# luxfi/tfhe

Measured on AMD Instinct MI355X. Metric: PBS/sec at TFHE 128-bit default (N=1024), batch=4096; 1/2/4/8 MI355X, higher is better.
Workload: dtype f64

## Files before the change

tfhe_amd/csrc/api.cpp:

```cpp
#include <dlfcn.h>
#include <hip/hip_runtime_api.h>
#include <rccl/rccl.h>
#include <stdarg.h>
#include <stdio.h>
#include <stdlib.h>
#include <string.h>

#include <algorithm>
#include <memory>
#include <mutex>
#include <string>
#include <thread>
#include <vector>

#include "../../include/tfhe_hip.h"
#include "client.h"
#include "gl64.h"
#include "pbs_kernels.h"

using tfhe::u32;
using tfhe::u64;

namespace {

// ... 54 lines not shown
}

struct Rccl {
  bool tried = false, ok = false;
  std::string why;
  ncclResult_t (*comm_init_all)(ncclComm_t*, int, const int*) = nullptr;
  ncclResult_t (*bcast)(const void*, void*, size_t, ncclDataType_t, int, ncclComm_t, hipStream_t) = nullptr;
  ncclResult_t (*group_start)() = nullptr;
  ncclResult_t (*group_end)() = nullptr;
  ncclResult_t (*comm_destroy)(ncclComm_t) = nullptr;
  const char* (*err)(ncclResult_t) = nullptr;
};

Rccl& rccl() {
  static Rccl r;
  static std::mutex m;
  std::lock_guard<std::mutex> lk(m);
  if (r.tried) return r;
  r.tried = true;
  void* h = dlopen("librccl.so.1", RTLD_NOW | RTLD_NOLOAD);
  if (!h) h = dlopen("librccl.so.1", RTLD_NOW | RTLD_LOCAL);
  if (!h) h = dlopen("/opt/rocm/lib/librccl.so.1", RTLD_NOW | RTLD_LOCAL);
  if (!h) {
    r.why = std::string("dlopen librccl.so.1: ") + dlerror();
    return r;
  }
  r.comm_init_all = (decltype(r.comm_init_all))dlsym(h, "ncclCommInitAll");
  r.bcast = (decltype(r.bcast))dlsym(h, "ncclBroadcast");
  r.group_start = (decltype(r.group_start))dlsym(h, "ncclGroupStart");
  r.group_end = (decltype(r.group_end))dlsym(h, "ncclGroupEnd");
  r.comm_destroy = (decltype(r.comm_destroy))dlsym(h, "ncclCommDestroy");
  r.err = (decltype(r.err))dlsym(h, "ncclGetErrorString");
  r.ok = r.comm_init_all && r.bcast && r.group_start && r.group_end && r.comm_destroy && r.err;
  if (!r.ok) r.why = "librccl.so.1 lacks ncclCommInitAll / ncclBroadcast / ncclGroupStart / ncclGroupEnd";
  return r;
}

struct DeviceGuard {
  int prev = -1;
  explicit DeviceGuard(int dev) {
    if (hipGetDevice(&prev) != hipSuccess) prev = -1;
    if (prev != dev) (void)hipSetDevice(dev);
  }
  ~DeviceGuard() {
    int cur = -1;
    if (prev >= 0 && hipGetDevice(&cur) == hipSuccess && cur != prev) (void)hipSetDevice(prev);
  }
};

}

struct tfhe_shard {
  int device = 0;
  hipStream_t stream = nullptr;
  u64* d_bsk = nullptr;
  u64* d_ksk = nullptr;
  void* d_ks_planes = nullptr;
  u64* d_tw = nullptr;
  u64* d_ms_zeros = nullptr;
  u64* d_big = nullptr;
  size_t big_cap = 0;
  void* d_stage = nullptr;
  size_t stage_cap = 0;
  void* d_ks_dig = nullptr;
  size_t ks_dig_cap = 0;
  hipEvent_t ws_free = nullptr;
  hipStream_t ws_last = nullptr;
  bool ws_used = false;
  std::vector<hipEvent_t> ev[3];
  std::vector<hipEvent_t> ev_pool;
};

struct tfhe_ctx {
  tfhe_params p{};
  std::vector<tfhe_shard> sh;
  bool keys = false;
  bool ks_valu = false;
  size_t lat_max = 1024;
  u64 ninv = 0;
  uint32_t ms_count = 0;
  double ms_bound = 0, ms_r_sigma = 0, ms_var128 = 0;
  int bcast_mode = 0;
  std::vector<ncclComm_t> comms;
  std::mutex mu;
  bool timing = false;
};

namespace {

using shard = tfhe_shard;

int grow(shard& s, void** ptr, size_t* cap, size_t bytes) {
  if (*cap >= bytes) return 0;
  if (s.ws_used) HIP_TRY(hipEventSynchronize(s.ws_free));
  if (*ptr) (void)hipFree(*ptr);
  *ptr = nullptr;
  *cap = 0;
  HIP_TRY(hipMalloc(ptr, bytes));
  *cap = bytes;
  return 0;
}

int ws_begin(shard& s, hipStream_t st) {
  if (s.ws_used && s.ws_last != st) HIP_TRY(hipStreamWaitEvent(st, s.ws_free, 0));
  return 0;
}
int ws_end(shard& s, hipStream_t st) {
  HIP_TRY(hipEventRecord(s.ws_free, st));
  s.ws_last = st;
  s.ws_used = true;
  return 0;
}

hipEvent_t take_event(shard& s) {
  if (!s.ev_pool.empty()) {
    hipEvent_t e = s.ev_pool.back();
    s.ev_pool.pop_back();
    return e;
  }
  hipEvent_t e = nullptr;
  if (hipEventCreate(&e) != hipSuccess) return nullptr;
  return e;
}

void timed_begin(tfhe_ctx* c, shard& s, int which, hipStream_t st) {
  if (!c->timing) return;
  hipEvent_t e = take_event(s);
  if (e) {
    (void)hipEventRecord(e, st);
    s.ev[which].push_back(e);
  }
}
void timed_end(tfhe_ctx* c, shard& s, int which, hipStream_t st) {
  if (!c->timing) return;
  if (s.ev[which].size() % 2 == 0) return;
  hipEvent_t e = take_event(s);
  if (e) {
    (void)hipEventRecord(e, st);
    s.ev[which].push_back(e);
  } else {
    s.ev_pool.push_back(s.ev[which].back());
    s.ev[which].pop_back();
  }
}

uint32_t io_dim(const tfhe_params& p) { return p.order == 0 ? p.n : p.k * p.N; }

hipError_t launch_br(tfhe_ctx* c, shard& s, const u64* in, size_t B, const u64* luts, const u32* idx, size_t n_lut,
                     u64* out_big, u64* out_acc, hipStream_t st) {
  if (is_fft(c->p) && c->p.N == 2048)
    return tfhe::launch_blind_rotate_fft2k(in, B, (int)c->p.n, luts, idx, (int)n_lut, (const double*)s.d_bsk,
                                           (const double*)s.d_tw, out_big, out_acc, st, c->lat_max);
  if (is_fft(c->p))
    return tfhe::launch_blind_rotate_fft(in, B, (int)c->p.n, luts, idx, (int)n_lut, (const double*)s.d_bsk,
                                         (const double*)s.d_tw, out_big, out_acc, st, c->lat_max);
  if (c->p.N == 2048)
    return tfhe::launch_blind_rotate_2048(in, B, (int)c->p.n, luts, idx, (int)n_lut, s.d_bsk, s.d_tw, out_big, out_acc,
                                          st, c->lat_max);
  return tfhe::launch_blind_rotate(in, B, (int)c->p.n, luts, idx, (int)n_lut, s.d_bsk, s.d_tw, out_big, out_acc, st,
                                   c->lat_max);
}

uint32_t log2u(uint32_t x) {
  uint32_t l = 0;
  while ((1u << l) < x) l++;
  return l;
}

hipError_t launch_ms(tfhe_ctx* c, shard& s, u64* small, size_t B, int* picks, hipStream_t st) {
  return tfhe::launch_ms_reduce(small, B, (int)c->p.n, s.d_ms_zeros, (int)c->ms_count, (int)log2u(2 * c->p.N),
                                c->ms_bound, c->ms_r_sigma, c->ms_var128, picks, st);
}

int launch_ks(tfhe_ctx* c, shard& s, const u64* in_big, size_t B, u64* out, hipStream_t st) {
  const int big_dim = (int)(c->p.k * c->p.N);
  if (c->ks_valu || !s.d_ks_planes) {
    HIP_TRY(tfhe::launch_keyswitch(in_big, B, big_dim, s.d_ksk, (int)c->p.n, (int)c->p.ks_base_log,
                                   (int)c->p.ks_level, out, st));
    return 0;
  }
  RC_TRY(grow(s, &s.d_ks_dig, &s.ks_dig_cap, tfhe::ks_digits_bytes(B, big_dim, (int)c->p.ks_level)));
  HIP_TRY(tfhe::launch_keyswitch_mfma(in_big, B, big_dim, s.d_ks_planes, (int)c->p.n, (int)c->p.ks_base_log,
                                      (int)c->p.ks_level, s.d_ks_dig, out, st));
  return 0;
}

int pbs_device(tfhe_ctx* c, shard& s, const u64* d_in, size_t B, const u64* d_luts, size_t n_lut, const u32* d_idx,
               u64* d_out, hipStream_t st) {
  const size_t big = (size_t)c->p.k * c->p.N + 1, small = (size_t)c->p.n + 1;
  RC_TRY(grow(s, (void**)&s.d_big, &s.big_cap, B * (c->p.order == 0 ? big : small) * sizeof(u64)));
  if (c->p.order == 0) {
    timed_begin(c, s, 0, st);
    HIP_TRY(launch_br(c, s, d_in, B, d_luts, d_idx, n_lut, s.d_big, nullptr, st));
    timed_end(c, s, 0, st);
    timed_begin(c, s, 1, st);
    RC_TRY(launch_ks(c, s, s.d_big, B, d_out, st));
    timed_end(c, s, 1, st);
  } else {
    timed_begin(c, s, 1, st);
    RC_TRY(launch_ks(c, s, d_in, B, s.d_big, st));
    timed_end(c, s, 1, st);
    if (c->ms_count) {
      timed_begin(c, s, 2, st);
      HIP_TRY(launch_ms(c, s, s.d_big, B, nullptr, st));
      timed_end(c, s, 2, st);
    }
    timed_begin(c, s, 0, st);
    HIP_TRY(launch_br(c, s, s.d_big, B, d_luts, d_idx, n_lut, d_out, nullptr, st));
// ... 128 lines not shown
      DeviceGuard g(c->sh[i].device);
      r = R->bcast(i == 0 ? (const void*)src : (const void*)dst[i], i == 0 ? (void*)src : (void*)dst[i], count,
                   ncclUint64, 0, c->comms[i], c->sh[i].stream);
    }
    const ncclResult_t r2 = R->group_end();
    if (r != ncclSuccess || r2 != ncclSuccess)
      return fail(TFHE_HIP_EDEVICE, "ncclBroadcast: %s", R->err(r != ncclSuccess ? r : r2));
    for (int i = 0; i < nd; i++) {
      DeviceGuard g(c->sh[i].device);
      HIP_TRY(hipStreamSynchronize(c->sh[i].stream));
    }
    c->bcast_mode = 2;
    return 0;
  }
  if (mode == 0) return 0;
  for (int k = 0; k < ncalls; k++) {
    shard& s = c->sh[calls[k]];
    DeviceGuard g(s.device);
    if (s.device == c->sh[0].device)
      HIP_TRY(hipMemcpyAsync(dst[calls[k]], src, count * 8, hipMemcpyDeviceToDevice, s.stream));
    else
      HIP_TRY(hipMemcpyPeerAsync(dst[calls[k]], s.device, src, c->sh[0].device, count * 8, s.stream));
    HIP_TRY(hipStreamSynchronize(s.stream));
  }
  c->bcast_mode = 1;
  return 0;
}

int convert_keys(tfhe_ctx* c, shard& s, const u64* std_bsk, size_t bsk_len) {
  const size_t polys = bsk_len / c->p.N;
  DeviceGuard g(s.device);
  if (!c->ks_valu) {
    const int big_dim = (int)(c->p.k * c->p.N);
    if (!s.d_ks_planes)
      HIP_TRY(hipMalloc(&s.d_ks_planes, tfhe::ks_planes_bytes(big_dim, (int)c->p.ks_level, (int)c->p.n)));
    HIP_TRY(tfhe::launch_ksk_planes(s.d_ksk, big_dim, (int)c->p.ks_level, (int)c->p.n, s.d_ks_planes, s.stream));
  }
  if (is_fft(c->p) && c->p.N == 2048)
    HIP_TRY(tfhe::launch_bsk_to_fourier2k(std_bsk, (double*)s.d_bsk, polys, (const double*)s.d_tw, s.stream));
  else if (is_fft(c->p))
    HIP_TRY(tfhe::launch_bsk_to_fourier(std_bsk, (double*)s.d_bsk, polys, (const double*)s.d_tw, s.stream));
  else if (c->p.N == 2048)
    HIP_TRY(tfhe::launch_bsk_to_ntt_2048(std_bsk, s.d_bsk, polys, s.d_tw, c->ninv, s.stream));
  else
    HIP_TRY(tfhe::launch_bsk_to_ntt(std_bsk, s.d_bsk, (int)(polys / 12), s.d_tw, c->ninv, s.stream));
  HIP_TRY(hipStreamSynchronize(s.stream));
  return 0;
}

int shard_init(tfhe_ctx* c, shard& s) {
  DeviceGuard g(s.device);
  HIP_TRY(hipStreamCreateWithFlags(&s.stream, hipStreamNonBlocking));
  HIP_TRY(hipEventCreateWithFlags(&s.ws_free, hipEventDisableTiming));
  const tfhe_params& p = c->p;
  using namespace tfhe;
  if (is_fft(p)) {
    std::vector<double> tw(p.N == 2048 ? fft2k_tables_len() : fft_tables_len());
    if (p.N == 2048) make_fft2k_tables(tw.data());
    else make_fft_tables(tw.data());
    if (!fft_slot_constants_ok() || !fft2k_slot_constants_ok())
      return fail(TFHE_HIP_EUNSUPPORTED, "FFT64: compile-time twist constants differ from the host tables");
    HIP_TRY(hipMalloc(&s.d_tw, tw.size() * 8));
    HIP_TRY(hipMemcpy(s.d_tw, tw.data(), tw.size() * 8, hipMemcpyHostToDevice));
    return 0;
  }
  std::vector<u64> tw(p.N == 2048 ? ntt2048_tables_len() : 4 * p.N);
  if (p.N == 2048) make_ntt2048_tables(canonical_psi(p.N), tw.data());
  else make_ntt_tables(canonical_psi(p.N), tw.data());
  HIP_TRY(hipMalloc(&s.d_tw, tw.size() * 8));
  HIP_TRY(hipMemcpy(s.d_tw, tw.data(), tw.size() * 8, hipMemcpyHostToDevice));
  return 0;
}

void shard_free(shard& s) {
  DeviceGuard g(s.device);
  if (s.stream) (void)hipStreamSynchronize(s.stream);
  for (int w = 0; w < 3; w++)
    for (auto e : s.ev[w]) (void)hipEventDestroy(e);
  for (auto e : s.ev_pool) (void)hipEventDestroy(e);
  (void)hipFree(s.d_bsk);
  (void)hipFree(s.d_ksk);
  (void)hipFree(s.d_ks_planes);
  (void)hipFree(s.d_ks_dig);
  (void)hipFree(s.d_tw);
  (void)hipFree(s.d_ms_zeros);
  (void)hipFree(s.d_big);
  (void)hipFree(s.d_stage);
  if (s.ws_free) (void)hipEventDestroy(s.ws_free);
  if (s.stream) (void)hipStreamDestroy(s.stream);
}

template <class F>
int for_each_slice(tfhe_ctx* c, size_t B, F&& fn) {
  const size_t nd = c->sh.size();
  std::vector<int> rc(nd, 0);
  std::vector<std::string> msg(nd);
  auto run = [&](size_t i) {
    const size_t lo = B * i / nd, hi = B * (i + 1) / nd;
    if (lo == hi) return;
    DeviceGuard g(c->sh[i].device);
    rc[i] = fn(i, lo, hi);
    if (rc[i]) msg[i] = g_err;
  };
  if (nd == 1) {
    run(0);
    return rc[0];
// ... 635 lines not shown
```

tfhe_amd/csrc/fft512.h:

```cpp
#pragma once
#pragma clang fp contract(off)
#include <hip/hip_runtime.h>

#include "gl64.h"
#include "ntt1024.h"

namespace tfhe {
namespace fftk {

constexpr int M = 512;
constexpr int S1 = 72, S2 = 65;
constexpr int T_C64 = 576;
constexpr int TW_TWIST = 0, TW_A = 512, TW_B = 1024, TW_I = 1536, TW_C64 = 2048;
constexpr double SQRT1_2 = 0.70710678118654752440;

#ifndef FFT_LDS_WAIT
#define FFT_LDS_WAIT 1
#endif
__device__ __forceinline__ void lds_order() {
#if FFT_LDS_WAIT
  wave_lds_sync();
#else
  __builtin_amdgcn_fence(__ATOMIC_ACQ_REL, "wavefront");
#endif
// ... 309 lines not shown
  for (int e = 0; e < 8; e++) {
    const double2 v = T[tb.b1 + 8 * e];
    xr[e] = v.x;
    xi[e] = v.y;
  }
  lds_order();
  dft8<false>(xr, xi);
#pragma unroll
  for (int e = 1; e < 8; e++) cmul<false>(xr[e], xi[e], wb[e]);
#pragma unroll
  for (int e = 0; e < 8; e++) T[lane + S2 * e] = make_double2(xr[e], xi[e]);
  lds_order();
#pragma unroll
  for (int e = 0; e < 8; e++) {
    const double2 v = T[tb.b2 + e];
    xr[e] = v.x;
    xi[e] = v.y;
  }
  lds_order();
  dft8<false>(xr, xi);
}

__device__ __forceinline__ void dft512_inv_rb(double (&xr)[8], double (&xi)[8], double2* T, int lane, TBase tb,
                                              const double2 (&wb)[8], const double2* twI) {
  dft8<true>(xr, xi);
#pragma unroll
  for (int e = 1; e < 8; e++) cmul<true>(xr[e], xi[e], wb[e]);
#pragma unroll
  for (int e = 0; e < 8; e++) T[tb.b2 + e] = make_double2(xr[e], xi[e]);
  lds_order();
#pragma unroll
  for (int e = 0; e < 8; e++) {
    const double2 v = T[lane + S2 * e];
    xr[e] = v.x;
    xi[e] = v.y;
  }
  lds_order();
  dft8<true>(xr, xi);
#pragma unroll
  for (int e = 0; e < 8; e++) cmul<true>(xr[e], xi[e], twI[64 * e + lane]);
#pragma unroll
  for (int e = 0; e < 8; e++) T[tb.b1 + 8 * e] = make_double2(xr[e], xi[e]);
  lds_order();
#pragma unroll
  for (int e = 0; e < 8; e++) {
    const double2 v = T[lane + S1 * e];
    xr[e] = v.x;
    xi[e] = v.y;
  }
  lds_order();
  dft8<true>(xr, xi);
}

template <bool TWIN = false, int BSTR = 8>
__device__ __forceinline__ void dft512_fwd_c(double (&xr)[8], double (&xi)[8], double2* T, int lane, TBase tb,
                                             const double2* twAl, const double2* twBc) {
  if constexpr (TWIN) twist_dft8_fwd(xr, xi);
  else dft8<false>(xr, xi);
#pragma unroll
  for (int e = 0; e < 8; e++) cmul<false>(xr[e], xi[e], twAl[64 * e]);
#pragma unroll
  for (int e = 0; e < 8; e++) T[lane + S1 * e] = make_double2(xr[e], xi[e]);
  lds_order();
#pragma unroll
  for (int e = 0; e < 8; e++) {
    const double2 v = T[tb.b1 + 8 * e];
    xr[e] = v.x;
    xi[e] = v.y;
  }
  lds_order();
  dft8<false>(xr, xi);
#pragma unroll
  for (int e = 1; e < 8; e++) cmul<false>(xr[e], xi[e], twBc[BSTR * e]);
#pragma unroll
  for (int e = 0; e < 8; e++) T[lane + S2 * e] = make_double2(xr[e], xi[e]);
  lds_order();
#pragma unroll
  for (int e = 0; e < 8; e++) {
    const double2 v = T[tb.b2 + e];
    xr[e] = v.x;
    xi[e] = v.y;
  }
  lds_order();
  dft8<false>(xr, xi);
}

template <int BSTR = 8>
__device__ __forceinline__ void dft512_inv_c(double (&xr)[8], double (&xi)[8], double2* T, int lane, TBase tb,
                                             const double2* twBc, const double2* twIl) {
  dft8<true>(xr, xi);
#pragma unroll
  for (int e = 1; e < 8; e++) cmul<true>(xr[e], xi[e], twBc[BSTR * e]);
#pragma unroll
  for (int e = 0; e < 8; e++) T[tb.b2 + e] = make_double2(xr[e], xi[e]);
  lds_order();
#pragma unroll
  for (int e = 0; e < 8; e++) {
    const double2 v = T[lane + S2 * e];
    xr[e] = v.x;
    xi[e] = v.y;
  }
  lds_order();
  dft8<true>(xr, xi);
#pragma unroll
  for (int e = 0; e < 8; e++) cmul<true>(xr[e], xi[e], twIl[64 * e]);
#pragma unroll
// ... 223 lines not shown
```

tfhe_amd/csrc/pbs_fft.hip:

```cpp
#pragma clang fp contract(off)
#include <hip/hip_runtime.h>

#include <type_traits>

#include "fft512.h"
#include "gl64.h"
#include "ntt1024.h"
#include "pbs_kernels.h"

namespace tfhe {
namespace fftk {

__device__ __forceinline__ void fft_fwd_real(const double (&a)[16], double (&xr)[8], double (&xi)[8], double2* T,
                                             int lane, const double2* tw) {
#pragma unroll
  for (int e = 0; e < 8; e++) {
    xr[e] = a[e];
    xi[e] = a[e + 8];
  }
  dft512_fwd<true, true>(xr, xi, T, lane, TBase(lane), tw);
}

__device__ __forceinline__ void fft_inv_real(double (&xr)[8], double (&xi)[8], double2* T, int lane, TBase tb,
                                             const double2* tw) {
// ... 50 lines not shown
                                                            const double2* __restrict__ tw) {
  __shared__ __attribute__((aligned(16))) double2 T[T_C64];
  const int lane = threadIdx.x;
  const size_t q = blockIdx.x;
  const u64* src = bsk_std + q * N1K;
  double a[16], xr[8], xi[8];
#pragma unroll
  for (int e = 0; e < 16; e++) a[e] = i64_to_f64(src[64 * e + lane]);
  fft_fwd_real(a, xr, xi, T, lane, tw);
  const size_t j = q % 2, r = (q / 2) % 6, i = q / 12;
  double2* dst = bsk_f + ((i * 6 + (r / 3) * 3 + (2 - r % 3)) * 2 + j) * M;
#pragma unroll
  for (int e = 0; e < 8; e++) dst[64 * e + lane] = make_double2(xr[e] * BSK_SCALE, xi[e] * BSK_SCALE);
}

__global__ __launch_bounds__(64) void fft_fwd_kernel(const u64* __restrict__ in, double2* __restrict__ out,
                                                     const double2* __restrict__ tw) {
  __shared__ __attribute__((aligned(16))) double2 T[T_C64];
  const int lane = threadIdx.x;
  const u64* src = in + (size_t)blockIdx.x * N1K;
  double a[16], xr[8], xi[8];
#pragma unroll
  for (int e = 0; e < 16; e++) a[e] = i64_to_f64(src[64 * e + lane]);
  fft_fwd_real(a, xr, xi, T, lane, tw);
  double2* dst = out + (size_t)blockIdx.x * M;
#pragma unroll
  for (int e = 0; e < 8; e++) dst[64 * e + lane] = make_double2(xr[e], xi[e]);
}

__global__ __launch_bounds__(64) void fft_inv_kernel(const double2* __restrict__ in, double* __restrict__ out,
                                                     const double2* __restrict__ tw) {
  __shared__ __attribute__((aligned(16))) double2 T[T_C64];
  const int lane = threadIdx.x;
  const double2* src = in + (size_t)blockIdx.x * M;
  double xr[8], xi[8];
#pragma unroll
  for (int e = 0; e < 8; e++) {
    const double2 v = src[64 * e + lane];
    xr[e] = v.x;
    xi[e] = v.y;
  }
  fft_inv_real(xr, xi, T, lane, TBase(lane), tw);
  double* dst = out + (size_t)blockIdx.x * N1K;
#pragma unroll
  for (int e = 0; e < 8; e++) {
    dst[64 * e + lane] = xr[e];
    dst[64 * (e + 8) + lane] = xi[e];
  }
}

#ifndef FFT_PRIO
#define FFT_PRIO 3
#endif

#ifndef FFT_ROT_BATCH
#define FFT_ROT_BATCH 0
#endif
#ifndef FFT_PAIR_TWREG
#define FFT_PAIR_TWREG 2
#endif
constexpr int STEP_C64 = 4 * M;
#ifndef FFT_PAIR_LDSTW
#define FFT_PAIR_LDSTW 1
#endif
template <int CTS, bool LDS_TW = (CTS == 4 && FFT_PAIR_LDSTW)>
struct FpShared {
  double2 tw[3 * M];
  double2 T[2 * CTS][T_C64];
  double2 K[2][STEP_C64];
};
template <int CTS>
struct FpShared<CTS, false> {
  double2 twI[M];
  double2 K[1][STEP_C64];
  double2 T[2 * CTS][T_C64];
};
#ifndef FFT_PAIR_CTS
#define FFT_PAIR_CTS 2
#endif
#ifndef FFT_MACPRIO
#define FFT_MACPRIO 1
#endif
#ifndef FFT_STAGGER
#define FFT_STAGGER 1
#endif
#ifndef FFT_TAILWG
#define FFT_TAILWG 256
#endif
#ifndef FFT_PRIO_SH
#define FFT_PRIO_SH 0
#endif
#ifndef FFT_ROTPRIO
#define FFT_ROTPRIO 0
#endif
#ifndef FFT_XCHPRIO
#define FFT_XCHPRIO 0
#endif
typedef __attribute__((address_space(3))) u64 lds_u64;

#ifndef FFT_ROT_UNIFORM
#define FFT_ROT_UNIFORM 1
#endif
__device__ __forceinline__ void rotate_states(const u64 (&v)[16], int a, int lane, double2* T, u32 (&st)[16]) {
  u64* Tu = (u64*)T;
#if FFT_ROT_UNIFORM
  a = __builtin_amdgcn_readfirstlane(a);
  const int A = (a >> 6) & 15, r = a & 63;
  const bool sgn = a >= 1024;
  {
    const u32 wb = (u32)(uintptr_t)(lds_u64*)&Tu[lane + r];
#pragma unroll
    for (int e = 0; e < 15; e++) ((lds_u64*)(uintptr_t)wb)[64 * e] = v[e];
    const bool w15 = lane + r >= 64;
    const u32 a15 = w15 ? wb + 960u * 8u - 8192u : wb + 960u * 8u;
    *(lds_u64*)(uintptr_t)a15 = w15 ? 0 - v[15] : v[15];
  }
  lds_order();
  const u32 rb = (u32)(uintptr_t)(lds_u64*)&Tu[lane] - 512u * (u32)A;
  const u32 wmask = (1u << A) - 1u;
  const u32 mbits = __builtin_amdgcn_readfirstlane(wmask ^ (sgn ? ~0u : 0u));
#pragma unroll
  for (int e = 0; e < 16; e++) {
    int m32;
    asm("s_bfe_i32 %0, %1, %2" : "=s"(m32) : "s"(mbits), "i"(e | (1 << 16)));
    const u64 M = (u64)(long long)m32;
    const u64 x = ((const lds_u64*)(uintptr_t)(rb + (__builtin_amdgcn_ubfe(wmask, e, 1) << 13)))[64 * e];
    st[e] = decomp_state((x ^ M) - (v[e] + M));
  }
  lds_order();
#else
#pragma unroll
  for (int e = 0; e < 16; e++) Tu[64 * e + lane] = v[e];
  lds_order();
  const int t0 = (lane - a) & 2047;
  const int u = t0 & 1023;
  const bool neg0 = t0 >= 1024;
  const u32 a0 = (u32)(uintptr_t)(lds_u64*)&Tu[u];
  const u32 a1 = a0 - 8192u;
#if FFT_ROT_BATCH
  u64 x[16];
#pragma unroll
  for (int e = 0; e < 16; e++) {
    const bool wrap = u >= 1024 - 64 * e;
    x[e] = ((const lds_u64*)(uintptr_t)(wrap ? a1 : a0))[64 * e];
  }
  __builtin_amdgcn_sched_barrier(0);
#pragma unroll
  for (int e = 0; e < 16; e++) {
    const bool neg = neg0 != (u >= 1024 - 64 * e);
    const u64 r = neg ? 0 - x[e] : x[e];
    st[e] = decomp_state(r - v[e]);
  }
#else
#pragma unroll
  for (int e = 0; e < 16; e++) {
    const bool wrap = u >= 1024 - 64 * e;
    const u32 base = wrap ? a1 : a0;
    const u64 x = ((const lds_u64*)(uintptr_t)base)[64 * e];
    const bool neg = neg0 != wrap;
    const u64 r = neg ? 0 - x : x;
    st[e] = decomp_state(r - v[e]);
  }
#endif
  lds_order();
#endif
}

template <int C>
__device__ __forceinline__ void exchange_partials(const double (&o0r)[8], const double (&o0i)[8], const double (&o1r)[8],
                                                  const double (&o1i)[8], double (&xr)[8], double (&xi)[8], double2* T,
                                                  const double2* Tp, int lane) {
#pragma unroll
  for (int e = 0; e < 8; e++) {
    T[64 * e + lane] = C ? make_double2(o0r[e], o0i[e]) : make_double2(o1r[e], o1i[e]);
    xr[e] = C ? o1r[e] : o0r[e];
    xi[e] = C ? o1i[e] : o0i[e];
  }
  __syncthreads();
#pragma unroll
  for (int e = 0; e < 8; e++) {
    const double2 w = Tp[64 * e + lane];
    xr[e] = xr[e] + w.x;
    xi[e] = xi[e] + w.y;
  }
  __syncthreads();
}

template <int NW>
__device__ __forceinline__ void load_step(const double2* __restrict__ bsk, int g, double2* dst, int wave_s, int lane) {
  const int i = g / 3, q = g - 3 * (g / 3);
#pragma unroll
  for (int u = 0; u < 32 / NW; u++) {
    const int blk = wave_s * (32 / NW) + u;
    const int c = blk >> 4;
    const char* src = (const char*)(bsk + ((size_t)i * 6 + c * 3 + q) * (2 * M)) + (blk & 15) * 1024;
    __builtin_amdgcn_global_load_lds((const void*)(src + lane * 16),
                                     (__attribute__((address_space(3))) void*)((char*)dst + blk * 1024), 16, 0, 0);
  }
}
#ifndef FFT_BUF_LDS
#define FFT_BUF_LDS 1
#endif
template <int NW>
__device__ __forceinline__ void load_step_buf(__amdgpu_buffer_rsrc_t bsr, int g, double2* dst, int wave_s, int voff) {
  const int i = g / 3, q = g - 3 * (g / 3);
#pragma unroll
  for (int u = 0; u < 32 / NW; u++) {
    const int blk = wave_s * (32 / NW) + u;
    const int c = blk >> 4;
    const int soff = ((i * 6 + c * 3 + q) * (2 * M)) * (int)sizeof(double2) + (blk & 15) * 1024;
    __builtin_amdgcn_raw_ptr_buffer_load_lds(bsr, (__attribute__((address_space(3))) void*)((char*)dst + blk * 1024),
                                             16, voff, soff, 0, 0);
  }
}

#ifndef FFT_WGTIME
#define FFT_WGTIME 0
#endif
#if FFT_WGTIME
__device__ unsigned long long g_wgt[4 * 16384];
#endif
template <int CTS, bool WRITE_ACC, bool WRITE_BIG>
__global__ __launch_bounds__(128 * CTS, 4 / CTS) void blind_rotate_fft_pair_kernel(
    const u64* __restrict__ lwe_in, int n, size_t B, const u64* __restrict__ luts, const u32* __restrict__ lut_index,
    int n_lut, const double2* __restrict__ bsk, const double2* __restrict__ tw_g, u64* __restrict__ out_big,
    u64* __restrict__ out_acc) {
  constexpr int NW = 2 * CTS;
  constexpr bool LDS_TW = CTS == 4 && FFT_PAIR_LDSTW;
  __shared__ __attribute__((aligned(16))) FpShared<CTS> sh;
#if FFT_WGTIME
  const unsigned long long wg_t0 = __builtin_amdgcn_s_memrealtime();
#endif
  const int wave = threadIdx.x >> 6, lane = threadIdx.x & 63;
  const int c = wave & 1;
  const size_t b_raw = (size_t)blockIdx.x * CTS + (wave >> 1);
  const bool live = b_raw < B;
  const size_t b = live ? b_raw : B - 1;
  const u64* ct = lwe_in + b * (size_t)(n + 1);
  double2* T = sh.T[wave];
  const double2* Tp = sh.T[wave ^ 1];
  const int wave_s = __builtin_amdgcn_readfirstlane(wave);
  const int c_s = wave_s & 1;
  const int n_steps = 3 * n;

#if FFT_BUF_LDS
  const __amdgpu_buffer_rsrc_t bsr =
      __builtin_amdgcn_make_buffer_rsrc((void*)bsk, (short)0, n * 6 * 2 * M * (int)sizeof(double2), 0x00020000);
  const int voff = lane * 16;
#endif
  if constexpr (LDS_TW) {
    for (int q = threadIdx.x; q < 3 * M; q += 64 * NW) sh.tw[q] = tw_g[TW_A + q];
    load_step<NW>(bsk, 0, sh.K[0], wave_s, lane);
  } else {
    for (int q = threadIdx.x; q < M; q += 64 * NW) sh.twI[q] = tw_g[TW_I + q];
  }

  u64 acc[16];
  {
    int li = lut_index ? (int)lut_index[b] : 0;
    li = (li < 0 || li >= n_lut) ? 0 : li;
    const u64* lut = luts + (size_t)li * N1K;
    const int s = (2048 - ms2048(ct[n])) & 2047;
#pragma unroll
    for (int e = 0; e < 16; e++) {
      int d = 64 * e + lane - s;
      bool neg = false;
      if (d < 0) { d += N1K; neg = !neg; }
      if (d < 0) { d += N1K; neg = !neg; }
      const u64 v = gl_to_torus(lut[d]);
      acc[e] = c ? (neg ? 0 - v : v) : 0;
    }
  }

  const TBase tb(lane);
  const double2* twA = tw_g + TW_A;
  const double2* twI;
  if constexpr (LDS_TW) {
    twA = sh.tw;
    twI = sh.tw + 2 * M;
  } else {
    twI = sh.twI;
  }
  const double2* twB = twA + M;
#if FFT_PAIR_TWREG
  double2 wa[8];
  __syncthreads();
#pragma unroll
  for (int e = 0; e < 8; e++) wa[e] = twA[64 * e + lane];
#endif
#if FFT_PAIR_TWREG >= 2
  double2 wb[8];
#pragma unroll
  for (int e = 1; e < 8; e++) wb[e] = twB[64 * e + lane];
  wb[0] = make_double2(1.0, 0.0);
#endif
#if FFT_PRIO == 1
  const bool prio_hi = NW > 4 && wave_s >= 4;
#elif FFT_PRIO == 3
  const bool prio_hi = (blockIdx.x >> 8) & 1;
#elif FFT_PRIO == 6
  [[maybe_unused]] constexpr bool prio_hi = false;
#elif FFT_PRIO == 5
  const bool prio_hi = ((blockIdx.x >> 8) ^ (blockIdx.x >> 9)) & 1;
#elif FFT_PRIO == 4
  const bool prio_hi = blockIdx.x + FFT_TAILWG >= gridDim.x;
#else
  constexpr bool prio_hi = false;
#endif
#if FFT_PRIO == 1 || FFT_PRIO == 0
  auto base_prio = [&]() {
    if (prio_hi) __builtin_amdgcn_s_setprio(1);
    else __builtin_amdgcn_s_setprio(0);
  };
#else
#if FFT_PRIO == 6
  const unsigned prio_ph = __builtin_amdgcn_readfirstlane((blockIdx.x >> 8) & 1);
  unsigned prio_flag = prio_ph;
#else
  const unsigned prio_flag = __builtin_amdgcn_readfirstlane(prio_hi ? 1u : 0u);
#endif
  auto base_prio = [&]() {
    asm volatile(
        "s_cmp_lg_u32 %0, 0\n\ts_cbranch_scc0 .Lbp0_%=\n\ts_setprio 1\n\ts_branch .Lbp1_%=\n"
        ".Lbp0_%=:\n\ts_setprio 0\n.Lbp1_%=:" ::"s"(prio_flag) : "scc");
  };
#endif
  base_prio();
#if FFT_STAGGER
  if (blockIdx.x < 512 && ((blockIdx.x >> 8) & 1))
    for (int k = 0; k < FFT_STAGGER; k++) __builtin_amdgcn_s_sleep(127);
#endif
  for (int i = 0; i < n; i++) {
#if FFT_PRIO == 6
    prio_flag = ((unsigned)i >> FFT_PRIO_SH ^ prio_ph) & 1u;
    base_prio();
#endif
    u32 st[16];
#if FFT_ROTPRIO
    __builtin_amdgcn_s_setprio(FFT_ROTPRIO);
#endif
    rotate_states(acc, ms2048(ct[i]), lane, T, st);
    double o0r[8], o0i[8], o1r[8], o1i[8];
    auto level = [&](auto qc) {
      constexpr int q = decltype(qc)::value;
      const int g = 3 * i + q;
#if FFT_MACPRIO
      if (q > 0 || FFT_ROTPRIO) base_prio();
#endif
      if constexpr (LDS_TW) {
        glds_barrier();
        if (g + 1 < n_steps) load_step<NW>(bsk, g + 1, sh.K[(g + 1) & 1], wave_s, lane);
      } else {
        if (q > 0) __syncthreads();
#if FFT_BUF_LDS
        load_step_buf<NW>(bsr, g, sh.K[0], wave_s, voff);
#else
        load_step<NW>(bsk, g, sh.K[0], wave_s, lane);
#endif
      }
      double xr[8], xi[8];
#pragma unroll
      for (int e = 0; e < 8; e++) {
        if constexpr (q == 2) {
          xr[e] = (double)decomp_top(st[e]);
          xi[e] = (double)decomp_top(st[e + 8]);
        } else {
          xr[e] = (double)decomp_step(st[e], 1u);
          xi[e] = (double)decomp_step(st[e + 8], 1u);
        }
      }
#if FFT_PAIR_TWREG >= 2
      dft512_fwd_rab<true>(xr, xi, T, lane, tb, wa, wb);
#elif FFT_PAIR_TWREG
      dft512_fwd_ra<true>(xr, xi, T, lane, tb, wa, twB);
#else
      dft512_fwd_t<true, true>(xr, xi, T, lane, tb, twA, twB);
#endif
      if constexpr (!LDS_TW) glds_barrier();
#if FFT_MACPRIO
      __builtin_amdgcn_s_setprio(3);
#endif
      const double2* k0 = sh.K[LDS_TW ? (g & 1) : 0] + c * (2 * M) + lane;
      const double2* k1 = k0 + M;
#pragma unroll
      for (int e = 0; e < 8; e++) {
        const double2 u = k0[64 * e], v = k1[64 * e];
        if constexpr (q == 0) {
          mac_first(o0r[e], o0i[e], xr[e], xi[e], u);
          mac_first(o1r[e], o1i[e], xr[e], xi[e], v);
        } else {
          mac_next(o0r[e], o0i[e], xr[e], xi[e], u);
          mac_next(o1r[e], o1i[e], xr[e], xi[e], v);
        }
      }
    };
    level(std::integral_constant<int, 0>{});
    level(std::integral_constant<int, 1>{});
    level(std::integral_constant<int, 2>{});
#if FFT_MACPRIO && !FFT_XCHPRIO
    base_prio();
#endif
    double xr[8], xi[8];
    if (c_s) exchange_partials<1>(o0r, o0i, o1r, o1i, xr, xi, T, Tp, lane);
    else exchange_partials<0>(o0r, o0i, o1r, o1i, xr, xi, T, Tp, lane);
#if FFT_MACPRIO && FFT_XCHPRIO
    base_prio();
#endif
#if FFT_PAIR_TWREG >= 2
    dft512_inv_rb(xr, xi, T, lane, tb, wb, twI);
#else
    dft512_inv_t(xr, xi, T, lane, tb, twB, twI);
#endif
    twist_slots<true>(xr, xi);
#pragma unroll
    for (int e = 0; e < 8; e++) {
      acc[e] = ACC_ADD(acc[e], xr[e]);
      acc[e + 8] = ACC_ADD(acc[e + 8], xi[e]);
    }
  }
#if FFT_WGTIME
  if (threadIdx.x == 0 && blockIdx.x < 16384) {
    const unsigned long long t1 = __builtin_amdgcn_s_memrealtime();
    g_wgt[4 * blockIdx.x] = wg_t0;
    g_wgt[4 * blockIdx.x + 1] = t1;
    g_wgt[4 * blockIdx.x + 2] = (unsigned)__builtin_amdgcn_s_getreg(4 | (31 << 11));
    g_wgt[4 * blockIdx.x + 3] = (unsigned)__builtin_amdgcn_s_getreg(20 | (31 << 11));
  }
#endif

  if (!live) return;
  if (WRITE_ACC) {
    u64* oa = out_acc + b * 2048 + c * N1K;
#pragma unroll
    for (int e = 0; e < 16; e++) oa[64 * e + lane] = acc[e];
  }
  if (WRITE_BIG) {
    u64* ob = out_big + b * (size_t)(N1K + 1);
    if (c == 0) {
#pragma unroll
      for (int e = 0; e < 16; e++) {
        const int idx = 64 * e + lane;
        if (idx == 0) ob[0] = acc[e];
        else ob[N1K - idx] = 0 - acc[e];
      }
    } else if (lane == 0) {
      ob[N1K] = acc[0];
    }
  }
}

#ifndef FFT_G3
#define FFT_G3 0
#endif
#ifndef G3_TW_GLOBAL
#define G3_TW_GLOBAL 0
#endif
constexpr int G3_CTS = 6;
constexpr int G3_NW = 2 * G3_CTS;
struct G3Shared {
  double2 twA[M];
  double2 twI[M];
// ... 389 lines not shown
static void twiddle(uint32_t t, uint32_t m, double* c, double* s) {
  t %= m;
  bool neg = false;
  if (2 * t > m) { t = m - t; neg = true; }
  double cc, ss;
  if (4 * t > m) {
    double cu, su;
    tw_quarter(t - m / 4, m, &cu, &su);
    cc = -su;
    ss = cu;
  } else {
    tw_quarter(t, m, &cc, &ss);
  }
  *c = cc;
  *s = neg ? -ss : ss;
}

}

void fft_twiddle(uint32_t t, uint32_t m, double* c, double* s) { fftk::twiddle(t, m, c, s); }

size_t fft_tables_len() { return 2 * fftk::TW_C64; }

void make_fft_tables(double* t) {
  using namespace fftk;
  for (uint32_t j = 0; j < (uint32_t)M; j++) twiddle(j, 4 * M, &t[2 * (TW_TWIST + j)], &t[2 * (TW_TWIST + j) + 1]);
  for (uint32_t e = 0; e < 8; e++)
    for (uint32_t L = 0; L < 64; L++) {
      twiddle((L * (1 + 4 * e)) % (4 * M), 4 * M, &t[2 * (TW_A + 64 * e + L)], &t[2 * (TW_A + 64 * e + L) + 1]);
      twiddle((8 * (L & 7) * e) % M, M, &t[2 * (TW_B + 64 * e + L)], &t[2 * (TW_B + 64 * e + L) + 1]);
      twiddle((((L & 7) + 8 * e) * (4 * (L >> 3) + 1)) % (4 * M), 4 * M, &t[2 * (TW_I + 64 * e + L)],
              &t[2 * (TW_I + 64 * e + L) + 1]);
    }
}

bool fft_slot_constants_ok() {
  for (int e = 0; e < 8; e++) {
    double c, s, c2, s2;
    fftk::twiddle(64u * e, 2048u, &c, &s);
    fftk::twiddle(128u * e, 4096u, &c2, &s2);
    if (c != fftk::ctw::SLOT[e].x || s != fftk::ctw::SLOT[e].y || c2 != c || s2 != s) return false;
  }
  return true;
}

hipError_t launch_bsk_to_fourier(const u64* bsk_std, double* bsk_f, size_t polys, const double* tw, hipStream_t s) {
  hipLaunchKernelGGL(fftk::bsk_to_fourier_kernel, dim3((unsigned)polys), dim3(64), 0, s, bsk_std, (double2*)bsk_f,
                     (const double2*)tw);
  return hipGetLastError();
}

hipError_t launch_blind_rotate_fft(const u64* lwe_in, size_t B, int n, const u64* luts, const u32* lut_index,
                                   int n_lut, const double* bsk_f, const double* tw, u64* out_big, u64* out_acc,
                                   hipStream_t s, size_t latency_max_batch) {
  using namespace fftk;
  if (B == 0) return hipSuccess;
  const double2 *bk = (const double2*)bsk_f, *t = (const double2*)tw;
  if (B <= latency_max_batch) {
    dim3 grid((unsigned)B), block(FL_THREADS);
    if (out_acc && out_big)
      hipLaunchKernelGGL((blind_rotate_fft_lat_kernel<true, true>), grid, block, 0, s, lwe_in, n, B, luts, lut_index,
                         n_lut, bk, t, out_big, out_acc);
    else if (out_acc)
      hipLaunchKernelGGL((blind_rotate_fft_lat_kernel<true, false>), grid, block, 0, s, lwe_in, n, B, luts, lut_index,
                         n_lut, bk, t, out_big, out_acc);
    else
      hipLaunchKernelGGL((blind_rotate_fft_lat_kernel<false, true>), grid, block, 0, s, lwe_in, n, B, luts, lut_index,
                         n_lut, bk, t, out_big, out_acc);
    return hipGetLastError();
  }
#if FFT_G3
  {
    int dev = 0, cus = 256;
    if (hipGetDevice(&dev) == hipSuccess) hipDeviceGetAttribute(&cus, hipDeviceAttributeMultiprocessorCount, dev);
    if (cus <= 0) cus = 256;
    const size_t rounds = (B + (size_t)G3_CTS * cus - 1) / ((size_t)G3_CTS * cus);
    size_t nwg = rounds * (size_t)cus;
    if (nwg > B) nwg = B;
    dim3 grid((unsigned)nwg), block(64 * G3_NW);
    if (out_acc && out_big)
      hipLaunchKernelGGL((blind_rotate_fft_g3_kernel<true, true>), grid, block, 0, s, lwe_in, n, B, luts, lut_index,
                         n_lut, bk, t, out_big, out_acc);
    else if (out_acc)
      hipLaunchKernelGGL((blind_rotate_fft_g3_kernel<true, false>), grid, block, 0, s, lwe_in, n, B, luts, lut_index,
                         n_lut, bk, t, out_big, out_acc);
    else
      hipLaunchKernelGGL((blind_rotate_fft_g3_kernel<false, true>), grid, block, 0, s, lwe_in, n, B, luts, lut_index,
                         n_lut, bk, t, out_big, out_acc);
    return hipGetLastError();
  }
#endif
  constexpr int CTS = FFT_PAIR_CTS;
  dim3 grid((unsigned)((B + CTS - 1) / CTS)), block(128 * CTS);
  if (out_acc && out_big)
    hipLaunchKernelGGL((blind_rotate_fft_pair_kernel<CTS, true, true>), grid, block, 0, s, lwe_in, n, B, luts,
                       lut_index, n_lut, bk, t, out_big, out_acc);
  else if (out_acc)
    hipLaunchKernelGGL((blind_rotate_fft_pair_kernel<CTS, true, false>), grid, block, 0, s, lwe_in, n, B, luts,
                       lut_index, n_lut, bk, t, out_big, out_acc);
  else
    hipLaunchKernelGGL((blind_rotate_fft_pair_kernel<CTS, false, true>), grid, block, 0, s, lwe_in, n, B, luts,
                       lut_index, n_lut, bk, t, out_big, out_acc);
  return hipGetLastError();
}

#if FFT_LATSTAMP
extern "C" int tfhe_hip_debug_latstamps(unsigned long long* out, size_t n) {
  if (n > 8 * 8 * 6) n = 8 * 8 * 6;
  return hipMemcpyFromSymbol(out, HIP_SYMBOL(fftk::g_latst), n * 8, 0, hipMemcpyDeviceToHost) == hipSuccess ? 0 : -1;
}
#endif
#if FFT_WGTIME
extern "C" int tfhe_hip_debug_wgtimes(unsigned long long* out, size_t n) {
  if (n > 4 * 16384) n = 4 * 16384;
  return hipMemcpyFromSymbol(out, HIP_SYMBOL(fftk::g_wgt), n * 8, 0, hipMemcpyDeviceToHost) == hipSuccess ? 0 : -1;
}
#endif

hipError_t launch_sample_extract_torus(const u64* acc, size_t B, u64* out, hipStream_t s) {
  if (B == 0) return hipSuccess;
  const size_t total = B * (N1K + 1);
  hipLaunchKernelGGL(fftk::sample_extract_torus_kernel, dim3((unsigned)((total + 255) / 256)), dim3(256), 0, s, acc, B,
                     out);
  return hipGetLastError();
}

hipError_t launch_fft_fwd(const u64* in, size_t count, double* out, const double* tw, hipStream_t s) {
  if (count == 0) return hipSuccess;
  hipLaunchKernelGGL(fftk::fft_fwd_kernel, dim3((unsigned)count), dim3(64), 0, s, in, (double2*)out,
                     (const double2*)tw);
  return hipGetLastError();
}

hipError_t launch_fft_inv(const double* in, size_t count, double* out, const double* tw, hipStream_t s) {
  if (count == 0) return hipSuccess;
  hipLaunchKernelGGL(fftk::fft_inv_kernel, dim3((unsigned)count), dim3(64), 0, s, (const double2*)in, out,
                     (const double2*)tw);
  return hipGetLastError();
}

}
```

tfhe_amd/csrc/pbs_kernels.h:

```cpp
#pragma once
#include <hip/hip_runtime.h>
#include <stddef.h>

#include "gl64.h"

namespace tfhe {
void make_ntt_tables(u64 psi, u64* tw);
hipError_t launch_bsk_to_ntt(const u64* bsk_std, u64* bsk_ntt, int n, const u64* tw, u64 ninv, hipStream_t s);
hipError_t launch_blind_rotate(const u64* lwe_in, size_t B, int n, const u64* luts, const u32* lut_index, int n_lut,
                               const u64* bsk, const u64* tw, u64* out_big, u64* out_acc, hipStream_t s,
                               size_t latency_max_batch = 0);
hipError_t launch_sample_extract(const u64* acc, size_t B, u64* out, hipStream_t s);
hipError_t launch_keyswitch(const u64* in_big, size_t B, int big_dim, const u64* ksk, int n, int base_log, int levels,
                           u64* out, hipStream_t s);
hipError_t launch_ntt_fwd(u64* polys, size_t count, const u64* tw, hipStream_t s);
hipError_t launch_ntt_inv(u64* polys, size_t count, const u64* tw, u64 ninv, hipStream_t s);
size_t ks_planes_bytes(int big_dim, int levels, int n);
size_t ks_digits_bytes(size_t B, int big_dim, int levels);
hipError_t launch_ksk_planes(const u64* ksk, int big_dim, int levels, int n, void* planes, hipStream_t s);
hipError_t launch_keyswitch_mfma(const u64* in_big, size_t B, int big_dim, const void* planes, int n, int base_log,
                                 int levels, void* digits, u64* out, hipStream_t s);

size_t fft_tables_len();
void make_fft_tables(double* tw);
bool fft_slot_constants_ok();
hipError_t launch_bsk_to_fourier(const u64* bsk_std, double* bsk_f, size_t polys, const double* tw, hipStream_t s);
hipError_t launch_blind_rotate_fft(const u64* lwe_in, size_t B, int n, const u64* luts, const u32* lut_index,
                                   int n_lut, const double* bsk_f, const double* tw, u64* out_big, u64* out_acc,
                                   hipStream_t s, size_t latency_max_batch = 0);
hipError_t launch_sample_extract_torus(const u64* acc, size_t B, u64* out, hipStream_t s);
hipError_t launch_fft_fwd(const u64* in, size_t count, double* out, const double* tw, hipStream_t s);
hipError_t launch_fft_inv(const double* in, size_t count, double* out, const double* tw, hipStream_t s);
size_t fft2k_tables_len();
void make_fft2k_tables(double* tw);
bool fft2k_slot_constants_ok();
hipError_t launch_bsk_to_fourier2k(const u64* bsk_std, double* bsk_f, size_t polys, const double* tw, hipStream_t s);
hipError_t launch_blind_rotate_fft2k(const u64* lwe_in, size_t B, int n, const u64* luts, const u32* lut_index,
                                     int n_lut, const double* bsk_f, const double* tw, u64* out_big, u64* out_acc,
                                     hipStream_t s, size_t latency_max_batch);
hipError_t launch_sample_extract_torus2k(const u64* acc, size_t B, u64* out, hipStream_t s);
hipError_t launch_fft2k_fwd(const u64* in, size_t count, double* out, const double* tw, hipStream_t s);
hipError_t launch_fft2k_inv(const double* in, size_t count, double* out, const double* tw, hipStream_t s);

void make_ntt2048_tables(u64 psi, u64* tw);
size_t ntt2048_tables_len();
hipError_t launch_bsk_to_ntt_2048(const u64* bsk_std, u64* bsk_ntt, size_t polys, const u64* tw, u64 ninv,
                                  hipStream_t s);
hipError_t launch_blind_rotate_2048(const u64* lwe_in, size_t B, int n, const u64* luts, const u32* lut_index,
                                   int n_lut, const u64* bsk, const u64* tw, u64* out_big, u64* out_acc,
                                   hipStream_t s, size_t latency_max_batch = 0);
hipError_t launch_sample_extract_2048(const u64* acc, size_t B, u64* out, hipStream_t s);
hipError_t launch_ntt2048_fwd(u64* polys, size_t count, const u64* tw, hipStream_t s);
size_t sns_fft_const_bytes();
void make_sns_fft_const(void* out);
size_t sns_fft_key_len(size_t n);
size_t sns_digit_len(size_t B);
size_t sns_fft_prod_len(size_t B);
constexpr size_t SNS_FFT_POLY_BYTES = 5 * 1024 * 16;
hipError_t launch_sns_bsk_to_fft(const u64* bsk_std, void* bsk_fft, size_t polys, const void* d_fconst,
                                 hipStream_t s);
hipError_t launch_sns_blind_rotate(const u64* lwe, size_t B, int n, const u64* lut, const void* bsk_fft, u64* acc,
                                   void* D, void* Oprod, const void* d_fconst, hipStream_t s);
hipError_t launch_sns_extract(const u64* acc, size_t B, u64* out, hipStream_t s);
hipError_t launch_pks_corr(const u64* pksk, int K, int Nc, int base_log, u64* corr, hipStream_t s);
hipError_t launch_pks_pack(const u64* lwes, size_t count, int in_dim, int base_log, int L, int k, int N, int lpg,
                           const u64* pksk, const u64* corr, u32* A, u64* T, u64* out, hipStream_t s);
size_t pks_mfma_rows(size_t count);
hipError_t launch_pks_gemm_mfma(const u64* lwes, size_t count, int in_dim, int base_log, int LV, int Nc,
                                const void* planes, void* A0, void* A1, u64* T, hipStream_t s);
hipError_t launch_pks_pack_mfma(const u64* lwes, size_t count, int in_dim, int base_log, int L, int k, int N, int lpg,
                                const void* planes, void* A0, void* A1, u64* T, u64* out, hipStream_t s);
inline size_t ms_zeros_pitch(size_t count) { return (count + 63) / 64 * 64; }
hipError_t launch_ms_reduce(u64* lwe, size_t B, int n, const u64* zeros, int count, int log2_2N, double bound,
                            double r_sigma, double var128, int* picks, hipStream_t s);
hipError_t launch_ntt2048_inv(u64* polys, size_t count, const u64* tw, u64 ninv, hipStream_t s);
}
```

Before: 176,800.

## Overlap FFT transpose twiddles with LDS stores, pipeline MAC loads, use CU count for priority

```diff
diff --git a/tfhe_amd/csrc/api.cpp b/tfhe_amd/csrc/api.cpp
--- a/tfhe_amd/csrc/api.cpp
+++ b/tfhe_amd/csrc/api.cpp
@@ -130,6 +130,7 @@
 
 struct tfhe_shard {
   int device = 0;
+  int cus = 0;
   hipStream_t stream = nullptr;
   u64* d_bsk = nullptr;
   u64* d_ksk = nullptr;
@@ -231,7 +232,7 @@
                                            (const double*)s.d_tw, out_big, out_acc, st, c->lat_max);
   if (is_fft(c->p))
     return tfhe::launch_blind_rotate_fft(in, B, (int)c->p.n, luts, idx, (int)n_lut, (const double*)s.d_bsk,
-                                         (const double*)s.d_tw, out_big, out_acc, st, c->lat_max);
+                                         (const double*)s.d_tw, out_big, out_acc, st, c->lat_max, s.cus);
   if (c->p.N == 2048)
     return tfhe::launch_blind_rotate_2048(in, B, (int)c->p.n, luts, idx, (int)n_lut, s.d_bsk, s.d_tw, out_big, out_acc,
                                           st, c->lat_max);
@@ -466,6 +467,7 @@
   DeviceGuard g(s.device);
   HIP_TRY(hipStreamCreateWithFlags(&s.stream, hipStreamNonBlocking));
   HIP_TRY(hipEventCreateWithFlags(&s.ws_free, hipEventDisableTiming));
+  HIP_TRY(hipDeviceGetAttribute(&s.cus, hipDeviceAttributeMultiprocessorCount, s.device));
   const tfhe_params& p = c->p;
   using namespace tfhe;
   if (is_fft(p)) {
diff --git a/tfhe_amd/csrc/fft512.h b/tfhe_amd/csrc/fft512.h
--- a/tfhe_amd/csrc/fft512.h
+++ b/tfhe_amd/csrc/fft512.h
@@ -385,6 +385,74 @@
   dft8<true>(xr, xi);
 }
 
+#ifndef FFT_XPOSE_OVERLAP
+#define FFT_XPOSE_OVERLAP 1
+#endif
+#ifndef FFT_XPOSE_NOWAIT
+#define FFT_XPOSE_NOWAIT 1
+#endif
+template <bool INV, int E0, int WS, int RS>
+__device__ __forceinline__ void xpose_p(double (&xr)[8], double (&xi)[8], const double2 (&w)[8], double2* Tw,
+                                        const double2* Tr) {
+#if FFT_XPOSE_OVERLAP
+#pragma unroll
+  for (int e = 0; e < 8; e++) {
+    if (e >= E0) cmul<INV>(xr[e], xi[e], w[e]);
+    Tw[WS * e] = make_double2(xr[e], xi[e]);
+    __builtin_amdgcn_sched_barrier(0);
+  }
+#else
+#pragma unroll
+  for (int e = E0; e < 8; e++) cmul<INV>(xr[e], xi[e], w[e]);
+#pragma unroll
+  for (int e = 0; e < 8; e++) Tw[WS * e] = make_double2(xr[e], xi[e]);
+#endif
+#if FFT_XPOSE_NOWAIT
+  __builtin_amdgcn_fence(__ATOMIC_ACQ_REL, "wavefront");
+  __builtin_amdgcn_sched_barrier(0);
+#pragma unroll
+  for (int k = 0; k < 8; k++) {
+    const int e = (k >> 1) + 4 * (k & 1);
+    const double2 v = Tr[RS * e];
+    xr[e] = v.x;
+    xi[e] = v.y;
+  }
+  __builtin_amdgcn_sched_barrier(0);
+#else
+  lds_order();
+#pragma unroll
+  for (int e = 0; e < 8; e++) {
+    const double2 v = Tr[RS * e];
+    xr[e] = v.x;
+    xi[e] = v.y;
+  }
+  lds_order();
+#endif
+}
+
+template <bool TWIN = false>
+__device__ __forceinline__ void dft512_fwd_rab_p(double (&xr)[8], double (&xi)[8], double2* T, int lane, TBase tb,
+                                                 const double2 (&wa)[8], const double2 (&wb)[8]) {
+  if constexpr (TWIN) twist_dft8_fwd(xr, xi);
+  else dft8<false>(xr, xi);
+  xpose_p<false, 0, S1, 8>(xr, xi, wa, T + lane, T + tb.b1);
+  dft8<false>(xr, xi);
+  xpose_p<false, 1, S2, 1>(xr, xi, wb, T + lane, T + tb.b2);
+  dft8<false>(xr, xi);
+}
+
+__device__ __forceinline__ void dft512_inv_rb_p(double (&xr)[8], double (&xi)[8], double2* T, int lane, TBase tb,
+                                                const double2 (&wb)[8], const double2* twI) {
+  dft8<true>(xr, xi);
+  xpose_p<true, 1, 1, S2>(xr, xi, wb, T + tb.b2, T + lane);
+  dft8<true>(xr, xi);
+  double2 wi[8];
+#pragma unroll
+  for (int e = 0; e < 8; e++) wi[e] = twI[64 * e + lane];
+  xpose_p<true, 0, 8, S1>(xr, xi, wi, T + tb.b1, T + lane);
+  dft8<true>(xr, xi);
+}
+
 template <bool TWIN = false, int BSTR = 8>
 __device__ __forceinline__ void dft512_fwd_c(double (&xr)[8], double (&xi)[8], double2* T, int lane, TBase tb,
                                              const double2* twAl, const double2* twBc) {
diff --git a/tfhe_amd/csrc/pbs_fft.hip b/tfhe_amd/csrc/pbs_fft.hip
--- a/tfhe_amd/csrc/pbs_fft.hip
+++ b/tfhe_amd/csrc/pbs_fft.hip
@@ -126,6 +126,21 @@
 #ifndef FFT_PRIO
 #define FFT_PRIO 3
 #endif
+constexpr unsigned dispatch_half(unsigned wg, unsigned cus) { return wg / cus; }
+constexpr bool wg_prio_hi(unsigned wg, unsigned cus) { return dispatch_half(wg, cus) & 1u; }
+constexpr bool wg_staggered(unsigned wg, unsigned cus) { return dispatch_half(wg, cus) == 1u; }
+namespace dh_check {
+constexpr bool same_as_bit8(unsigned n) {
+  for (unsigned w = 0; w < n; w++)
+    if (wg_prio_hi(w, 256) != (((w >> 8) & 1u) != 0) || wg_staggered(w, 256) != (w < 512 && ((w >> 8) & 1u))) return false;
+  return true;
+}
+static_assert(same_as_bit8(4096), "dispatch_half(., 256) must reproduce the 256-CU split");
+static_assert(!wg_prio_hi(31, 32) && wg_prio_hi(32, 32) && wg_prio_hi(63, 32) && !wg_prio_hi(64, 32) && wg_prio_hi(96, 32), "32 CUs");
+static_assert(!wg_staggered(31, 32) && wg_staggered(32, 32) && wg_staggered(63, 32) && !wg_staggered(64, 32) && !wg_staggered(96, 32), "32 CUs");
+static_assert(!wg_prio_hi(303, 304) && wg_prio_hi(304, 304) && wg_prio_hi(607, 304) && !wg_prio_hi(608, 304) && wg_prio_hi(912, 304), "304 CUs");
+static_assert(!wg_staggered(303, 304) && wg_staggered(304, 304) && wg_staggered(607, 304) && !wg_staggered(608, 304) && !wg_staggered(912, 304), "304 CUs");
+}
 
 #ifndef FFT_ROT_BATCH
 #define FFT_ROT_BATCH 0
@@ -170,6 +185,12 @@
 #ifndef FFT_XCHPRIO
 #define FFT_XCHPRIO 0
 #endif
+#ifndef FFT_MAC_PIPE
+#define FFT_MAC_PIPE 1
+#endif
+#ifndef FFT_MAC_PIPE_Q2
+#define FFT_MAC_PIPE_Q2 (FFT_MAC_PIPE ? 2 : 0)
+#endif
 typedef __attribute__((address_space(3))) u64 lds_u64;
 
 #ifndef FFT_ROT_UNIFORM
@@ -240,7 +261,7 @@
 #endif
 }
 
-template <int C>
+template <int C, bool GROUP = false>
 __device__ __forceinline__ void exchange_partials(const double (&o0r)[8], const double (&o0i)[8], const double (&o1r)[8],
                                                   const double (&o1i)[8], double (&xr)[8], double (&xi)[8], double2* T,
                                                   const double2* Tp, int lane) {
@@ -251,11 +272,24 @@
     xi[e] = C ? o1i[e] : o0i[e];
   }
   __syncthreads();
-#pragma unroll
-  for (int e = 0; e < 8; e++) {
-    const double2 w = Tp[64 * e + lane];
-    xr[e] = xr[e] + w.x;
-    xi[e] = xi[e] + w.y;
+  if constexpr (GROUP) {
+    double2 w[8];
+    __builtin_amdgcn_sched_barrier(0);
+#pragma unroll
+    for (int e = 0; e < 8; e++) w[e] = Tp[64 * e + lane];
+    __builtin_amdgcn_sched_barrier(0);
+#pragma unroll
+    for (int e = 0; e < 8; e++) {
+      xr[e] = xr[e] + w[e].x;
+      xi[e] = xi[e] + w[e].y;
+    }
+  } else {
+#pragma unroll
+    for (int e = 0; e < 8; e++) {
+      const double2 w = Tp[64 * e + lane];
+      xr[e] = xr[e] + w.x;
+      xi[e] = xi[e] + w.y;
+    }
   }
   __syncthreads();
 }
@@ -298,7 +332,7 @@
 __global__ __launch_bounds__(128 * CTS, 4 / CTS) void blind_rotate_fft_pair_kernel(
     const u64* __restrict__ lwe_in, int n, size_t B, const u64* __restrict__ luts, const u32* __restrict__ lut_index,
     int n_lut, const double2* __restrict__ bsk, const double2* __restrict__ tw_g, u64* __restrict__ out_big,
-    u64* __restrict__ out_acc) {
+    u64* __restrict__ out_acc, int n_cus) {
   constexpr int NW = 2 * CTS;
   constexpr bool LDS_TW = CTS == 4 && FFT_PAIR_LDSTW;
   __shared__ __attribute__((aligned(16))) FpShared<CTS> sh;
@@ -371,7 +405,7 @@
 #if FFT_PRIO == 1
   const bool prio_hi = NW > 4 && wave_s >= 4;
 #elif FFT_PRIO == 3
-  const bool prio_hi = (blockIdx.x >> 8) & 1;
+  const bool prio_hi = wg_prio_hi(blockIdx.x, (unsigned)n_cus);
 #elif FFT_PRIO == 6
   [[maybe_unused]] constexpr bool prio_hi = false;
 #elif FFT_PRIO == 5
@@ -401,7 +435,7 @@
 #endif
   base_prio();
 #if FFT_STAGGER
-  if (blockIdx.x < 512 && ((blockIdx.x >> 8) & 1))
+  if (wg_staggered(blockIdx.x, (unsigned)n_cus))
     for (int k = 0; k < FFT_STAGGER; k++) __builtin_amdgcn_s_sleep(127);
 #endif
   for (int i = 0; i < n; i++) {
@@ -443,7 +477,9 @@
           xi[e] = (double)decomp_step(st[e + 8], 1u);
         }
       }
-#if FFT_PAIR_TWREG >= 2
+#if FFT_PAIR_TWREG >= 2 && (FFT_XPOSE_OVERLAP || FFT_XPOSE_NOWAIT)
+      dft512_fwd_rab_p<true>(xr, xi, T, lane, tb, wa, wb);
+#elif FFT_PAIR_TWREG >= 2
       dft512_fwd_rab<true>(xr, xi, T, lane, tb, wa, wb);
 #elif FFT_PAIR_TWREG
       dft512_fwd_ra<true>(xr, xi, T, lane, tb, wa, twB);
@@ -456,6 +492,29 @@
 #endif
       const double2* k0 = sh.K[LDS_TW ? (g & 1) : 0] + c * (2 * M) + lane;
       const double2* k1 = k0 + M;
+#if FFT_MAC_PIPE
+      if constexpr (q > 0) {
+        constexpr int D = q == 2 ? FFT_MAC_PIPE_Q2 : FFT_MAC_PIPE;
+        double2 ku[8], kv[8];
+#pragma unroll
+        for (int e = 0; e < D; e++) {
+          ku[e] = k0[64 * e];
+          kv[e] = k1[64 * e];
+        }
+#pragma unroll
+        for (int e = 0; e < 8; e++) {
+          if (e + D < 8) {
+            ku[e + D] = k0[64 * (e + D)];
+            kv[e + D] = k1[64 * (e + D)];
+          }
+          __builtin_amdgcn_sched_barrier(0);
+          mac_next(o0r[e], o0i[e], xr[e], xi[e], ku[e]);
+          mac_next(o1r[e], o1i[e], xr[e], xi[e], kv[e]);
+          __builtin_amdgcn_sched_barrier(0);
+        }
+        return;
+      }
+#endif
 #pragma unroll
       for (int e = 0; e < 8; e++) {
         const double2 u = k0[64 * e], v = k1[64 * e];
@@ -475,12 +534,14 @@
     base_prio();
 #endif
     double xr[8], xi[8];
-    if (c_s) exchange_partials<1>(o0r, o0i, o1r, o1i, xr, xi, T, Tp, lane);
-    else exchange_partials<0>(o0r, o0i, o1r, o1i, xr, xi, T, Tp, lane);
+    if (c_s) exchange_partials<1, FFT_XPOSE_OVERLAP != 0>(o0r, o0i, o1r, o1i, xr, xi, T, Tp, lane);
+    else exchange_partials<0, FFT_XPOSE_OVERLAP != 0>(o0r, o0i, o1r, o1i, xr, xi, T, Tp, lane);
 #if FFT_MACPRIO && FFT_XCHPRIO
     base_prio();
 #endif
-#if FFT_PAIR_TWREG >= 2
+#if FFT_PAIR_TWREG >= 2 && (FFT_XPOSE_OVERLAP || FFT_XPOSE_NOWAIT)
+    dft512_inv_rb_p(xr, xi, T, lane, tb, wb, twI);
+#elif FFT_PAIR_TWREG >= 2
     dft512_inv_rb(xr, xi, T, lane, tb, wb, twI);
 #else
     dft512_inv_t(xr, xi, T, lane, tb, twB, twI);
@@ -976,9 +1037,10 @@
 
 hipError_t launch_blind_rotate_fft(const u64* lwe_in, size_t B, int n, const u64* luts, const u32* lut_index,
                                    int n_lut, const double* bsk_f, const double* tw, u64* out_big, u64* out_acc,
-                                   hipStream_t s, size_t latency_max_batch) {
+                                   hipStream_t s, size_t latency_max_batch, int n_cus) {
   using namespace fftk;
   if (B == 0) return hipSuccess;
+  if (n_cus <= 0) n_cus = 256;
   const double2 *bk = (const double2*)bsk_f, *t = (const double2*)tw;
   if (B <= latency_max_batch) {
     dim3 grid((unsigned)B), block(FL_THREADS);
@@ -1018,13 +1080,13 @@
   dim3 grid((unsigned)((B + CTS - 1) / CTS)), block(128 * CTS);
   if (out_acc && out_big)
     hipLaunchKernelGGL((blind_rotate_fft_pair_kernel<CTS, true, true>), grid, block, 0, s, lwe_in, n, B, luts,
-                       lut_index, n_lut, bk, t, out_big, out_acc);
+                       lut_index, n_lut, bk, t, out_big, out_acc, n_cus);
   else if (out_acc)
     hipLaunchKernelGGL((blind_rotate_fft_pair_kernel<CTS, true, false>), grid, block, 0, s, lwe_in, n, B, luts,
-                       lut_index, n_lut, bk, t, out_big, out_acc);
+                       lut_index, n_lut, bk, t, out_big, out_acc, n_cus);
   else
     hipLaunchKernelGGL((blind_rotate_fft_pair_kernel<CTS, false, true>), grid, block, 0, s, lwe_in, n, B, luts,
-                       lut_index, n_lut, bk, t, out_big, out_acc);
+                       lut_index, n_lut, bk, t, out_big, out_acc, n_cus);
   return hipGetLastError();
 }
 
diff --git a/tfhe_amd/csrc/pbs_kernels.h b/tfhe_amd/csrc/pbs_kernels.h
--- a/tfhe_amd/csrc/pbs_kernels.h
+++ b/tfhe_amd/csrc/pbs_kernels.h
@@ -27,7 +27,7 @@
 hipError_t launch_bsk_to_fourier(const u64* bsk_std, double* bsk_f, size_t polys, const double* tw, hipStream_t s);
 hipError_t launch_blind_rotate_fft(const u64* lwe_in, size_t B, int n, const u64* luts, const u32* lut_index,
                                    int n_lut, const double* bsk_f, const double* tw, u64* out_big, u64* out_acc,
-                                   hipStream_t s, size_t latency_max_batch = 0);
+                                   hipStream_t s, size_t latency_max_batch = 0, int n_cus = 0);
 hipError_t launch_sample_extract_torus(const u64* acc, size_t B, u64* out, hipStream_t s);
 hipError_t launch_fft_fwd(const u64* in, size_t count, double* out, const double* tw, hipStream_t s);
 hipError_t launch_fft_inv(const double* in, size_t count, double* out, const double* tw, hipStream_t s);
```

Result: faster. 179,100, median of 6 (+1.3%).
